# seanrjohnson/protein_gibbs_sampler

Measured on AMD Instinct MI355X. Metric: sampled positions/sec (whole node), ESM-1b L=256 B=256 Gibbs, higher is better.
Workload: dtype bf16

## Files before the change

protein_gibbs_sampler_amd/csrc/attention.hip:

```cpp
#include <stdlib.h>

#include "kernels.h"

PG_OPS_BEGIN

typedef __attribute__((ext_vector_type(8))) __bf16 bf16x8;
typedef __attribute__((ext_vector_type(4))) float f32x4;
typedef __attribute__((ext_vector_type(2))) float f32x2;

typedef short v4s __attribute__((ext_vector_type(4)));

#ifdef PG_ATT_PROF
__device__ unsigned long long* pg_att_prof;
#define PG_T(slot, i)                                                                                              \
  do {                                                                                                             \
    if ((slot) < 8 && (threadIdx.x & 63) == 0)                                                                     \
      pg_att_prof[(((size_t)blockIdx.x * 4 + (threadIdx.x >> 6)) * 8 + (slot)) * 8 + (i)] = __builtin_readcyclecounter(); \
  } while (0)
#else
#define PG_T(slot, i)
#endif

template <int MAXKB, bool PADMASK, bool BIASKV = false, bool SPLIT = false>
__global__ __launch_bounds__(256, (MAXKB <= 18 ? 2 : 1)) void attention_kernel(const bf16_t* __restrict__ qkv, bf16_t* __restrict__ ctx, int T,
                                                       int H, int ld_qkv_, int ld_ctx_, int k_off, int v_off,
                                                       SeqLayout sl, const int32_t* __restrict__ key_tok, int pad_idx,
                                                       const bf16_t* __restrict__ bias_kv, int split_from = 0, int split = 1) {
  __shared__ __attribute__((aligned(16))) char smem[2 * MAXKB * 16 * 128 + (PADMASK ? MAXKB * 16 : 0)];
  char* Ks = smem;
  char* Vs = smem + MAXKB * 16 * 128;
  char* padf = smem + 2 * MAXKB * 16 * 128;

  const int tid = threadIdx.x, lane = tid & 63, wave = tid >> 6;
  PG_T(7, 0);
  int pair = blockIdx.x, qb_first = wave, qb_step = 4;
  if (SPLIT && (int)blockIdx.x >= split_from) {
    const int u = blockIdx.x - split_from;
    pair = split_from + u / split;
    qb_first = u % split + split * wave;
    qb_step = 4 * split;
  }
  const int seq = pair / H, h = pair % H;
  const size_t row0 = (size_t)(seq / sl.inner_count) * sl.outer_rows + (size_t)(seq % sl.inner_count) * sl.inner_rows;
  const size_t ld_qkv = (size_t)ld_qkv_ * sl.row_step, ld_ctx = (size_t)ld_ctx_ * sl.row_step;
  const bf16_t* base = qkv + row0 * ld_qkv_ + h * 64;
  const int Tk = T + (BIASKV ? 1 : 0);
  constexpr int nkc = MAXKB / 2;
  constexpr int tpad = MAXKB * 16;

  {
    constexpr int NIT = (MAXKB * 16 * 8 + 255) / 256;
    uint4 kreg[NIT], vreg[NIT];
#pragma unroll
    for (int it = 0; it < NIT; ++it) {
      const int i = tid + it * 256;
      const int row = i >> 3, c = i & 7;
      kreg[it] = make_uint4(0, 0, 0, 0);
      vreg[it] = make_uint4(0, 0, 0, 0);
      if (i < tpad * 8 && row < T) {
        kreg[it] = *(const uint4*)(base + (size_t)row * ld_qkv + k_off + c * 8);
        vreg[it] = *(const uint4*)(base + (size_t)row * ld_qkv + v_off + c * 8);
      } else if (BIASKV && row == T) {
        kreg[it] = *(const uint4*)(bias_kv + h * 64 + c * 8);
        vreg[it] = *(const uint4*)(bias_kv + (H + h) * 64 + c * 8);
      }
    }
#pragma unroll
    for (int it = 0; it < NIT; ++it) {
      const int i = tid + it * 256;
      if (i < tpad * 8) {
        const int row = i >> 3, c = i & 7;
        *(uint4*)(Ks + row * 128 + ((c ^ (row & 7)) << 4)) = kreg[it];
        *(uint4*)(Vs + row * 128 + ((c ^ (row & 7)) << 4)) = vreg[it];
      }
    }
  }
  if (PADMASK) {
    for (int key = tid; key < MAXKB * 16; key += 256)
      padf[key] = (key < T && key_tok[row0 + (size_t)key * sl.row_step] == pad_idx) ? 1 : 0;
  }
  PG_T(7, 1);
  __syncthreads();
  PG_T(7, 2);

  const int fr = lane & 15, fq = lane >> 4;
  const int nqb = (T + 15) >> 4;
  bf16x8 qf[2], qn[2];
  auto load_q = [&](int qb, bf16x8 (&dst)[2]) {
    int qrow = qb * 16 + fr;
    if (qrow >= T) qrow = T - 1;
#pragma unroll
    for (int kk = 0; kk < 2; ++kk) dst[kk] = *(const bf16x8*)(base + (size_t)qrow * ld_qkv + kk * 32 + fq * 8);
  };
  if (qb_first < nqb) load_q(qb_first, qf);
  for (int qb = qb_first; qb < nqb; qb += qb_step) {
    if (qb + qb_step < nqb) load_q(qb + qb_step, qn);
    PG_T(qb >> 2, 0);

    f32x4 st[MAXKB];
    {
      constexpr int CH = (MAXKB % 6 == 0) ? 6 : (MAXKB % 4 == 0 ? 4 : 2);
      bf16x8 kbuf[2][CH][2];
      auto load_chunk = [&](int ch, bf16x8 (&dst)[CH][2]) {
#pragma unroll
        for (int u = 0; u < CH; ++u) {
#if defined(PG_ATT_PROF) && PG_ATT_ABL == 1
          const int krow = (ch * CH + (u > 0 ? 0 : u)) * 16 + fr;
          if (u > 0) { dst[u][0] = dst[0][0]; dst[u][1] = dst[0][1]; continue; }
#else
          const int krow = (ch * CH + u) * 16 + fr;
#endif
#pragma unroll
          for (int kk = 0; kk < 2; ++kk) dst[u][kk] = *(const bf16x8*)(Ks + krow * 128 + (((kk * 4 + fq) ^ (krow & 7)) << 4));
        }
      };
      load_chunk(0, kbuf[0]);
#pragma unroll
      for (int ch = 0; ch < MAXKB / CH; ++ch) {
        if (ch + 1 < MAXKB / CH) load_chunk(ch + 1, kbuf[(ch + 1) & 1]);
        __builtin_amdgcn_sched_barrier(0);
#pragma unroll
        for (int u = 0; u < CH; ++u)
          st[ch * CH + u] = mfma_op16(kbuf[ch & 1][u][0], qf[0], (f32x4){0.f, 0.f, 0.f, 0.f});
#pragma unroll
        for (int u = 0; u < CH; ++u)
          st[ch * CH + u] = mfma_op16(kbuf[ch & 1][u][1], qf[1], st[ch * CH + u]);
        __builtin_amdgcn_sched_barrier(0);
      }
    }
    PG_T(qb >> 2, 1);
    float mx = -3.0e38f;
    int tl = Tk - fq * 4;
    asm volatile("" : "+v"(tl));
#pragma unroll
    for (int kb = MAXKB > 6 ? MAXKB - 6 : 0; kb < MAXKB; ++kb)
      if ((kb + 1) * 16 > Tk) {
#pragma unroll
        for (int r = 0; r < 4; ++r)
          if (kb * 16 + r >= tl) st[kb][r] = -3.0e38f;
      }
#pragma unroll
    for (int kb = 0; kb < MAXKB; ++kb)
#pragma unroll
      for (int r = 0; r < 4; ++r) mx = fmaxf(mx, st[kb][r]);
    if (PADMASK) {
      const float fill = sl.row_step == 1 ? -3.0e38f : -10000.0f;
      mx = -3.0e38f;
#pragma unroll
      for (int kb = 0; kb < MAXKB; ++kb) {
        const uint32_t f4 = *(const uint32_t*)(padf + kb * 16 + fq * 4);
#pragma unroll
        for (int r = 0; r < 4; ++r) {
          if ((f4 >> (8 * r)) & 0xffu) st[kb][r] = fill;
          mx = fmaxf(mx, st[kb][r]);
        }
      }
    }
    mx = rows4_max(mx);
    const f32x2 l2e = {1.44269504088896341f, 1.44269504088896341f};
    const float mneg1 = -mx * 1.44269504088896341f;
    const f32x2 mneg = {mneg1, mneg1};
    f32x2 sum2 = {0.f, 0.f};
#pragma unroll
    for (int kb = 0; kb < MAXKB; ++kb) {
      const f32x2 a = __builtin_elementwise_fma((f32x2){st[kb][0], st[kb][1]}, l2e, mneg);
      const f32x2 b = __builtin_elementwise_fma((f32x2){st[kb][2], st[kb][3]}, l2e, mneg);
      const f32x2 ea = {__builtin_amdgcn_exp2f(a[0]), __builtin_amdgcn_exp2f(a[1])};
      const f32x2 eb = {__builtin_amdgcn_exp2f(b[0]), __builtin_amdgcn_exp2f(b[1])};
      st[kb] = (f32x4){ea[0], ea[1], eb[0], eb[1]};
      sum2 += ea;
      sum2 += eb;
    }
    float sum = sum2[0] + sum2[1];
    sum = rows4_sum(sum);
    const float inv = 1.0f / sum;
    PG_T(qb >> 2, 2);

    f32x4 o[4];
#pragma unroll
    for (int db = 0; db < 4; ++db) o[db] = (f32x4){0.f, 0.f, 0.f, 0.f};
    {
      union VF { bf16x8 v; uint2 h[2]; };
      VF vbuf[3][4];
      auto load_v = [&](int c, VF (&dst)[4]) {
#pragma unroll
        for (int db = 0; db < 4; ++db) {
#if defined(PG_ATT_PROF) && PG_ATT_ABL == 2
          if (db > 0) { dst[db] = dst[0]; continue; }
#endif
#pragma unroll
          for (int hh = 0; hh < 2; ++hh) {
            const int krow = (2 * c + hh) * 16 + fq * 4 + (fr >> 2);
            const int dcol = db * 16 + (fr & 3) * 4;
            const char* a = Vs + krow * 128 + (((dcol >> 3) ^ (krow & 7)) << 4) + ((dcol >> 2) & 1) * 8;
            const v4s t = __builtin_amdgcn_ds_read_tr16_b64_v4i16((v4s __attribute__((address_space(3)))*)(
                (__attribute__((address_space(3))) char*)a));
            dst[db].h[hh] = __builtin_bit_cast(uint2, t);
          }
        }
      };
      load_v(0, vbuf[0]);
      if (nkc > 1) load_v(1, vbuf[1]);
#pragma unroll
      for (int c = 0; c < nkc; ++c) {
        if (c + 2 < nkc) load_v(c + 2, vbuf[(c + 2) % 3]);
        union { bf16x8 v; uint32_t u[4]; } pf;
        const f32x4 lo = st[2 * c], hi = st[2 * c + 1];
        pf.u[0] = pack_op2(lo[0], lo[1]);
        pf.u[1] = pack_op2(lo[2], lo[3]);
        pf.u[2] = pack_op2(hi[0], hi[1]);
        pf.u[3] = pack_op2(hi[2], hi[3]);
        __builtin_amdgcn_sched_barrier(0);
#pragma unroll
        for (int db = 0; db < 4; ++db) o[db] = mfma_op16(vbuf[c % 3][db].v, pf.v, o[db]);
        __builtin_amdgcn_sched_barrier(0);
      }
    }
    PG_T(qb >> 2, 3);
    const int q = qb * 16 + fr;
    if (q < T) {
      bf16_t* dst = ctx + row0 * ld_ctx_ + (size_t)q * ld_ctx + h * 64 + fq * 4;
#pragma unroll
      for (int db = 0; db < 4; ++db) {
        uint2 p;
        p.x = pack_op2(o[db][0] * inv, o[db][1] * inv);
        p.y = pack_op2(o[db][2] * inv, o[db][3] * inv);
        *(uint2*)(dst + db * 16) = p;
      }
    }
    qf[0] = qn[0];
    qf[1] = qn[1];
    PG_T(qb >> 2, 4);
  }
  PG_T(7, 3);
}

template <int MAXKB, int OCC, bool PADMASK, bool BIASKV>
__global__ __launch_bounds__(256, OCC) void attention_long_kernel(const bf16_t* __restrict__ qkv, bf16_t* __restrict__ ctx, int T,
                                                               int H, int ld_qkv_, int ld_ctx_, int k_off, int v_off,
                                                               SeqLayout sl, int n_qchunk, const int32_t* __restrict__ key_tok_,
                                                               int pad_idx, const bf16_t* __restrict__ bias_kv_) {
  const int32_t* __restrict__ key_tok = PADMASK ? key_tok_ : nullptr;
  const bf16_t* __restrict__ bias_kv = BIASKV ? bias_kv_ : nullptr;
  constexpr int tpad = MAXKB * 16, nkc = MAXKB / 2;
  __shared__ __attribute__((aligned(16))) char smem[2 * tpad * 128 + (PADMASK ? tpad : 0)];
  char* Ks = smem;
  char* Vs = smem + tpad * 128;
  char* padf = smem + 2 * tpad * 128;
  const int tid = threadIdx.x, lane = tid & 63, wave = tid >> 6;
  const int qc = blockIdx.x % n_qchunk, sh = blockIdx.x / n_qchunk;
  const int seq = sh / H, h = sh % H;
  const size_t row0 = (size_t)(seq / sl.inner_count) * sl.outer_rows + (size_t)(seq % sl.inner_count) * sl.inner_rows;
  const size_t ld_qkv = (size_t)ld_qkv_ * sl.row_step, ld_ctx = (size_t)ld_ctx_ * sl.row_step;
  const bf16_t* base = qkv + row0 * ld_qkv_ + h * 64;
  const int fr = lane & 15, fq = lane >> 4;
  const int q0 = qc * 64 + wave * 16;
  const bool active = q0 < T;
  bf16x8 qf[2];
  {
    int qrow = q0 + fr;
    if (qrow >= T) qrow = T - 1;
#pragma unroll
    for (int kk = 0; kk < 2; ++kk) qf[kk] = *(const bf16x8*)(base + (size_t)qrow * ld_qkv + kk * 32 + fq * 8);
  }
  f32x4 o[4];
#pragma unroll
  for (int db = 0; db < 4; ++db) o[db] = (f32x4){0.f, 0.f, 0.f, 0.f};
  float m = -3.0e38f, l = 0.f;
  constexpr float LOG2E = 1.44269504088896341f;
  const int Tk = T + (bias_kv ? 1 : 0);

  for (int k0 = 0; k0 < Tk; k0 += tpad) {
    __syncthreads();
    {
      constexpr int NIT = (tpad * 8 + 255) / 256;
      uint4 kreg[NIT], vreg[NIT];
#pragma unroll
      for (int it = 0; it < NIT; ++it) {
        const int i = tid + it * 256, row = i >> 3, c = i & 7;
        kreg[it] = make_uint4(0, 0, 0, 0);
        vreg[it] = make_uint4(0, 0, 0, 0);
        if (i < tpad * 8 && k0 + row < T) {
          kreg[it] = *(const uint4*)(base + (size_t)(k0 + row) * ld_qkv + k_off + c * 8);
          vreg[it] = *(const uint4*)(base + (size_t)(k0 + row) * ld_qkv + v_off + c * 8);
        } else if (bias_kv && k0 + row == T) {
          kreg[it] = *(const uint4*)(bias_kv + h * 64 + c * 8);
          vreg[it] = *(const uint4*)(bias_kv + (H + h) * 64 + c * 8);
        }
      }
#pragma unroll
      for (int it = 0; it < NIT; ++it) {
        const int i = tid + it * 256, row = i >> 3, c = i & 7;
        if (i < tpad * 8) {
          *(uint4*)(Ks + row * 128 + ((c ^ (row & 7)) << 4)) = kreg[it];
          *(uint4*)(Vs + row * 128 + ((c ^ (row & 7)) << 4)) = vreg[it];
        }
      }
    }
    if (PADMASK) {
      for (int key = tid; key < tpad; key += 256)
        padf[key] = (k0 + key < T && key_tok[row0 + (size_t)(k0 + key) * sl.row_step] == pad_idx) ? 1 : 0;
    }
    __syncthreads();
    if (!active) continue;
    f32x4 st[MAXKB];
#pragma unroll
    for (int kb = 0; kb < MAXKB; ++kb) {
      st[kb] = (f32x4){0.f, 0.f, 0.f, 0.f};
      const int krow = kb * 16 + fr;
#pragma unroll
      for (int kk = 0; kk < 2; ++kk) {
        const bf16x8 kf = *(const bf16x8*)(Ks + krow * 128 + (((kk * 4 + fq) ^ (krow & 7)) << 4));
        st[kb] = mfma_op16(kf, qf[kk], st[kb]);
      }
    }
    float tmax = -3.0e38f;
    const int tl = Tk - k0 - fq * 4;
#pragma unroll
    for (int kb = 0; kb < MAXKB; ++kb)
#pragma unroll
      for (int r = 0; r < 4; ++r) {
        if (kb * 16 + r >= tl) st[kb][r] = -3.0e38f;
        tmax = fmaxf(tmax, st[kb][r]);
      }
    if (PADMASK) {
      const float fill = sl.row_step == 1 ? -3.0e38f : -10000.0f;
      tmax = -3.0e38f;
#pragma unroll
      for (int kb = 0; kb < MAXKB; ++kb) {
        const uint32_t f4 = *(const uint32_t*)(padf + kb * 16 + fq * 4);
#pragma unroll
        for (int r = 0; r < 4; ++r) {
          if ((f4 >> (8 * r)) & 0xffu) st[kb][r] = fill;
          tmax = fmaxf(tmax, st[kb][r]);
        }
      }
    }
    tmax = rows4_max(tmax);
    const float mn = fmaxf(m, tmax);
    const float alpha = __builtin_amdgcn_exp2f((m - mn) * LOG2E);
    const float mneg = -mn * LOG2E;
    float psum = 0.f;
#pragma unroll
    for (int kb = 0; kb < MAXKB; ++kb)
#pragma unroll
      for (int r = 0; r < 4; ++r) {
        const float e = __builtin_amdgcn_exp2f(fmaf(st[kb][r], LOG2E, mneg));
        st[kb][r] = e;
        psum += e;
      }
    psum = rows4_sum(psum);
    l = l * alpha + psum;
    m = mn;
#pragma unroll
    for (int db = 0; db < 4; ++db) {
      o[db][0] *= alpha; o[db][1] *= alpha; o[db][2] *= alpha; o[db][3] *= alpha;
    }
#pragma unroll
    for (int c = 0; c < nkc; ++c) {
      union { bf16x8 v; uint32_t u[4]; } pf;
      const f32x4 lo = st[2 * c], hi = st[2 * c + 1];
      pf.u[0] = pack_op2(lo[0], lo[1]);
      pf.u[1] = pack_op2(lo[2], lo[3]);
      pf.u[2] = pack_op2(hi[0], hi[1]);
      pf.u[3] = pack_op2(hi[2], hi[3]);
#pragma unroll
      for (int db = 0; db < 4; ++db) {
        union { bf16x8 v; uint2 h2[2]; } vf;
#pragma unroll
        for (int hh = 0; hh < 2; ++hh) {
          const int krow = (2 * c + hh) * 16 + fq * 4 + (fr >> 2);
          const int dcol = db * 16 + (fr & 3) * 4;
          const char* a = Vs + krow * 128 + (((dcol >> 3) ^ (krow & 7)) << 4) + ((dcol >> 2) & 1) * 8;
          vf.h2[hh] = __builtin_bit_cast(uint2, __builtin_amdgcn_ds_read_tr16_b64_v4i16((v4s __attribute__((address_space(3)))*)(
                                                    (__attribute__((address_space(3))) char*)a)));
        }
        o[db] = mfma_op16(vf.v, pf.v, o[db]);
      }
    }
  }
  const int q = q0 + fr;
  if (active && q < T) {
    const float inv = 1.0f / l;
    bf16_t* dst = ctx + row0 * ld_ctx_ + (size_t)q * ld_ctx + h * 64 + fq * 4;
#pragma unroll
    for (int db = 0; db < 4; ++db) {
      uint2 p;
      p.x = pack_op2(o[db][0] * inv, o[db][1] * inv);
      p.y = pack_op2(o[db][2] * inv, o[db][3] * inv);
      *(uint2*)(dst + db * 16) = p;
    }
  }
}

int launch_attention_bf16(hipStream_t s, const bf16_t* qkv, bf16_t* ctx, int B, int T, int H, int ld_qkv, int ld_ctx,
                          int k_off, int v_off, const int32_t* key_tok, int pad_idx, const bf16_t* bias_kv) {
  SeqLayout sl = {1, T, 0, 1};
  return launch_attention_seq_bf16(s, qkv, ctx, B, T, H, ld_qkv, ld_ctx, k_off, v_off, sl, key_tok, pad_idx, bias_kv);
}

int launch_attention_seq_bf16(hipStream_t s, const bf16_t* qkv, bf16_t* ctx, int64_t n_seq, int T, int H, int ld_qkv,
                              int ld_ctx, int k_off, int v_off, SeqLayout sl, const int32_t* key_tok, int pad_idx,
                              const bf16_t* bias_kv) {
  if (n_seq == 0) return 0;
  if (n_seq * H > 0x7fffffff) return fail(1, "attention: too many sequences");
  dim3 grid((unsigned)(n_seq * H)), block(256);
  static const int split_on = [] { const char* e = getenv("PGIBBS_ATTN_SPLIT"); return e ? atoi(e) : 1; }();
  static const int n_cu = [] { hipDeviceProp_t p; int d = 0; (void)hipGetDevice(&d); return hipGetDeviceProperties(&p, d) == hipSuccess ? p.multiProcessorCount : 256; }();
  int split_from = 0, split = 1;
  if (split_on && !key_tok && !bias_kv && sl.row_step == 1 && T >= 64 && T <= 576) {
    const int kb = (((T + 15) / 16) + 1) & ~1;
    const long pairs = n_seq * H, slots = (long)n_cu * (kb <= 20 ? 2 : 1);
    const long rem = pairs % slots;
    const int nqb = (T + 15) / 16;
    int sp = rem ? (int)(slots / rem) : 1;
    if (sp > 4) sp = 4;
    if (sp > nqb / 4) sp = nqb / 4;
    if (sp >= 2) {
      split = sp;
      split_from = (int)(pairs - rem);
      grid = dim3((unsigned)(split_from + rem * sp));
    }
  }
#define PG_ATT_SPLIT_LAUNCH(KB) hipLaunchKernelGGL((attention_kernel<KB, false, false, true>), grid, block, 0, s, qkv, ctx, T, H, ld_qkv, ld_ctx, k_off, v_off, sl, key_tok, pad_idx, bias_kv, split_from, split)
#define PG_ATT(KB)                                                                                             \
  else if (Tk <= KB * 16) {                                                                                    \
    if (bias_kv && key_tok) hipLaunchKernelGGL((attention_kernel<KB, true, true>), grid, block, 0, s, qkv, ctx, T, H, ld_qkv, ld_ctx, k_off, v_off, sl, key_tok, pad_idx, bias_kv); \
    else if (bias_kv) hipLaunchKernelGGL((attention_kernel<KB, false, true>), grid, block, 0, s, qkv, ctx, T, H, ld_qkv, ld_ctx, k_off, v_off, sl, key_tok, pad_idx, bias_kv); \
    else if (key_tok) hipLaunchKernelGGL((attention_kernel<KB, true>), grid, block, 0, s, qkv, ctx, T, H, ld_qkv, ld_ctx, k_off, v_off, sl, key_tok, pad_idx, bias_kv); \
    else if (split > 1) PG_ATT_SPLIT_LAUNCH(KB);                                                               \
    else hipLaunchKernelGGL((attention_kernel<KB, false>), grid, block, 0, s, qkv, ctx, T, H, ld_qkv, ld_ctx, k_off, v_off, sl, key_tok, pad_idx, bias_kv); \
  }
  const int Tk = T + (bias_kv ? 1 : 0);
  static const int fine_ladder = [] { const char* e = getenv("PGIBBS_ATTN_LADDER"); return e ? atoi(e) : 1; }();
  if (T <= 0) return fail(1, "attention: empty sequence");
#define PG_ATT_PLAIN(KB)                                                                                       \
  else if (fine_ladder && !bias_kv && Tk <= KB * 16) {                                                         \
    if (key_tok) hipLaunchKernelGGL((attention_kernel<KB, true>), grid, block, 0, s, qkv, ctx, T, H, ld_qkv, ld_ctx, k_off, v_off, sl, key_tok, pad_idx, bias_kv); \
    else if (split > 1) PG_ATT_SPLIT_LAUNCH(KB);                                                               \
    else hipLaunchKernelGGL((attention_kernel<KB, false>), grid, block, 0, s, qkv, ctx, T, H, ld_qkv, ld_ctx, k_off, v_off, sl, key_tok, pad_idx, bias_kv); \
  }
  PG_ATT(2) PG_ATT(4) PG_ATT_PLAIN(6) PG_ATT(8) PG_ATT_PLAIN(10) PG_ATT(12) PG_ATT_PLAIN(14) PG_ATT_PLAIN(16) PG_ATT(18)
  PG_ATT_PLAIN(20) PG_ATT_PLAIN(22) PG_ATT(24) PG_ATT_PLAIN(26) PG_ATT_PLAIN(28) PG_ATT(30) PG_ATT_PLAIN(32) PG_ATT_PLAIN(34) PG_ATT(36)
#undef PG_ATT_PLAIN
#undef PG_ATT
#undef PG_ATT_SPLIT_LAUNCH
  else {
    const int n_qchunk = (T + 63) / 64;
    if (n_seq * H * n_qchunk > 0x7fffffff) return fail(1, "attention: too many sequences");
    const dim3 g((unsigned)(n_seq * H * n_qchunk));
#define PG_ATT_LONG(P, B) hipLaunchKernelGGL((attention_long_kernel<18, 2, P, B>), g, block, 0, s, qkv, ctx, T, H, ld_qkv, ld_ctx, k_off, v_off, sl, n_qchunk, key_tok, pad_idx, bias_kv)
    if (key_tok && bias_kv) PG_ATT_LONG(true, true);
    else if (key_tok) PG_ATT_LONG(true, false);
    else if (bias_kv) PG_ATT_LONG(false, true);
    else PG_ATT_LONG(false, false);
#undef PG_ATT_LONG
  }
  PG_HIP(hipGetLastError());
  return 0;
}

PG_OPS_END
```

Baseline: 72010.

## Process two query blocks per wave in attention to reuse K/V fragment loads

Refactors the attention body into a templated pass that handles NQ query blocks at once, and adds a PAIR kernel variant in which each wave computes two 16-row query blocks per pass. Each K and V fragment read from LDS then feeds two MFMAs. The next pair's Q loads are issued after the score computation. The pair path is the default for unmasked, no-bias sequences with 14 to 28 key blocks, which includes L=256. In exchange it roughly doubles the score and accumulator registers, which risks spills or lower occupancy (launch bounds are adjusted for this), and it interacts with the existing split-block scheduling.

```diff
diff --git a/protein_gibbs_sampler_amd/csrc/attention.hip b/protein_gibbs_sampler_amd/csrc/attention.hip
--- a/protein_gibbs_sampler_amd/csrc/attention.hip
+++ b/protein_gibbs_sampler_amd/csrc/attention.hip
@@ -21,8 +21,183 @@
 #define PG_T(slot, i)
 #endif
 
-template <int MAXKB, bool PADMASK, bool BIASKV = false, bool SPLIT = false>
-__global__ __launch_bounds__(256, (MAXKB <= 18 ? 2 : 1)) void attention_kernel(const bf16_t* __restrict__ qkv, bf16_t* __restrict__ ctx, int T,
+template <int MAXKB, bool PADMASK, bool BIASKV, int NQ, class AfterS>
+__device__ __forceinline__ void attention_pass(const char* Ks, const char* Vs, const char* padf, bf16x8 (&qf)[2][2], const int (&qb)[2],
+                                               int slot, int T, int Tk, float padfill, bf16_t* ctx_head, size_t ld_ctx,
+                                               AfterS after_s) {
+  const int lane = threadIdx.x & 63, fr = lane & 15, fq = lane >> 4;
+  constexpr int nkc = MAXKB / 2;
+  PG_T(slot, 0);
+
+  f32x4 st[NQ][MAXKB];
+  {
+#if defined(PG_ATT_PROF) && defined(PG_ATT_PAIR_CH)
+    constexpr int CH = NQ == 2 ? (MAXKB == 18 ? PG_ATT_PAIR_CH : 2) : ((MAXKB % 6 == 0) ? 6 : (MAXKB % 4 == 0 ? 4 : 2));
+#else
+    constexpr int CH = NQ == 2 ? (MAXKB % 6 == 0 ? 3 : 2) : ((MAXKB % 6 == 0) ? 6 : (MAXKB % 4 == 0 ? 4 : 2));
+#endif
+    static_assert(MAXKB % CH == 0, "whole chunks");
+    bf16x8 kbuf[2][CH][2];
+    auto load_chunk = [&](int ch, bf16x8 (&dst)[CH][2]) {
+#pragma unroll
+      for (int u = 0; u < CH; ++u) {
+#if defined(PG_ATT_PROF) && PG_ATT_ABL == 1
+        const int krow = (ch * CH + (u > 0 ? 0 : u)) * 16 + fr;
+        if (u > 0) { dst[u][0] = dst[0][0]; dst[u][1] = dst[0][1]; continue; }
+#else
+        const int krow = (ch * CH + u) * 16 + fr;
+#endif
+#pragma unroll
+        for (int kk = 0; kk < 2; ++kk) dst[u][kk] = *(const bf16x8*)(Ks + krow * 128 + (((kk * 4 + fq) ^ (krow & 7)) << 4));
+      }
+    };
+    load_chunk(0, kbuf[0]);
+#pragma unroll
+    for (int ch = 0; ch < MAXKB / CH; ++ch) {
+      if (ch + 1 < MAXKB / CH) load_chunk(ch + 1, kbuf[(ch + 1) & 1]);
+      __builtin_amdgcn_sched_barrier(0);
+#pragma unroll
+      for (int u = 0; u < CH; ++u)
+#pragma unroll
+        for (int n = 0; n < NQ; ++n)
+          st[n][ch * CH + u] = mfma_op16(kbuf[ch & 1][u][0], qf[n][0], (f32x4){0.f, 0.f, 0.f, 0.f});
+#pragma unroll
+      for (int u = 0; u < CH; ++u)
+#pragma unroll
+        for (int n = 0; n < NQ; ++n)
+          st[n][ch * CH + u] = mfma_op16(kbuf[ch & 1][u][1], qf[n][1], st[n][ch * CH + u]);
+      __builtin_amdgcn_sched_barrier(0);
+    }
+  }
+  PG_T(slot, 1);
+  after_s();
+  float mx[NQ];
+  int tl = Tk - fq * 4;
+  asm volatile("" : "+v"(tl));
+#pragma unroll
+  for (int n = 0; n < NQ; ++n) {
+    mx[n] = -3.0e38f;
+#pragma unroll
+    for (int kb = MAXKB > 6 ? MAXKB - 6 : 0; kb < MAXKB; ++kb)
+      if ((kb + 1) * 16 > Tk) {
+#pragma unroll
+        for (int r = 0; r < 4; ++r)
+          if (kb * 16 + r >= tl) st[n][kb][r] = -3.0e38f;
+      }
+#pragma unroll
+    for (int kb = 0; kb < MAXKB; ++kb)
+#pragma unroll
+      for (int r = 0; r < 4; ++r) mx[n] = fmaxf(mx[n], st[n][kb][r]);
+    if (PADMASK) {
+      mx[n] = -3.0e38f;
+#pragma unroll
+      for (int kb = 0; kb < MAXKB; ++kb) {
+        const uint32_t f4 = *(const uint32_t*)(padf + kb * 16 + fq * 4);
+#pragma unroll
+        for (int r = 0; r < 4; ++r) {
+          if ((f4 >> (8 * r)) & 0xffu) st[n][kb][r] = padfill;
+          mx[n] = fmaxf(mx[n], st[n][kb][r]);
+        }
+      }
+    }
+    mx[n] = rows4_max(mx[n]);
+  }
+  const f32x2 l2e = {1.44269504088896341f, 1.44269504088896341f};
+  f32x2 mneg[NQ], sum2[NQ];
+#pragma unroll
+  for (int n = 0; n < NQ; ++n) {
+    const float mneg1 = -mx[n] * 1.44269504088896341f;
+    mneg[n] = (f32x2){mneg1, mneg1};
+    sum2[n] = (f32x2){0.f, 0.f};
+  }
+#pragma unroll
+  for (int kb = 0; kb < MAXKB; ++kb)
+#pragma unroll
+    for (int n = 0; n < NQ; ++n) {
+      const f32x2 a = __builtin_elementwise_fma((f32x2){st[n][kb][0], st[n][kb][1]}, l2e, mneg[n]);
+      const f32x2 b = __builtin_elementwise_fma((f32x2){st[n][kb][2], st[n][kb][3]}, l2e, mneg[n]);
+      const f32x2 ea = {__builtin_amdgcn_exp2f(a[0]), __builtin_amdgcn_exp2f(a[1])};
+      const f32x2 eb = {__builtin_amdgcn_exp2f(b[0]), __builtin_amdgcn_exp2f(b[1])};
+      st[n][kb] = (f32x4){ea[0], ea[1], eb[0], eb[1]};
+      sum2[n] += ea;
+      sum2[n] += eb;
+    }
+  float inv[NQ];
+#pragma unroll
+  for (int n = 0; n < NQ; ++n) {
+    float sum = sum2[n][0] + sum2[n][1];
+    sum = rows4_sum(sum);
+    inv[n] = 1.0f / sum;
+  }
+  PG_T(slot, 2);
+
+  f32x4 o[NQ][4];
+#pragma unroll
+  for (int n = 0; n < NQ; ++n)
+#pragma unroll
+    for (int db = 0; db < 4; ++db) o[n][db] = (f32x4){0.f, 0.f, 0.f, 0.f};
+  {
+    constexpr int VD = (NQ == 2 && MAXKB == 20) ? 2 : 3;
+    union VF { bf16x8 v; uint2 h[2]; };
+    VF vbuf[VD][4];
+    auto load_v = [&](int c, VF (&dst)[4]) {
+#pragma unroll
+      for (int db = 0; db < 4; ++db) {
+#if defined(PG_ATT_PROF) && PG_ATT_ABL == 2
+        if (db > 0) { dst[db] = dst[0]; continue; }
+#endif
+#pragma unroll
+        for (int hh = 0; hh < 2; ++hh) {
+          const int krow = (2 * c + hh) * 16 + fq * 4 + (fr >> 2);
+          const int dcol = db * 16 + (fr & 3) * 4;
+          const char* a = Vs + krow * 128 + (((dcol >> 3) ^ (krow & 7)) << 4) + ((dcol >> 2) & 1) * 8;
+          const v4s t = __builtin_amdgcn_ds_read_tr16_b64_v4i16((v4s __attribute__((address_space(3)))*)(
+              (__attribute__((address_space(3))) char*)a));
+          dst[db].h[hh] = __builtin_bit_cast(uint2, t);
+        }
+      }
+    };
+    load_v(0, vbuf[0]);
+    if (VD > 2 && nkc > 1) load_v(1, vbuf[1]);
+#pragma unroll
+    for (int c = 0; c < nkc; ++c) {
+      if (c + VD - 1 < nkc) load_v(c + VD - 1, vbuf[(c + VD - 1) % VD]);
+      union { bf16x8 v; uint32_t u[4]; } pf[NQ];
+#pragma unroll
+      for (int n = 0; n < NQ; ++n) {
+        const f32x4 lo = st[n][2 * c], hi = st[n][2 * c + 1];
+        pf[n].u[0] = pack_op2(lo[0], lo[1]);
+        pf[n].u[1] = pack_op2(lo[2], lo[3]);
+        pf[n].u[2] = pack_op2(hi[0], hi[1]);
+        pf[n].u[3] = pack_op2(hi[2], hi[3]);
+      }
+      __builtin_amdgcn_sched_barrier(0);
+#pragma unroll
+      for (int db = 0; db < 4; ++db)
+#pragma unroll
+        for (int n = 0; n < NQ; ++n) o[n][db] = mfma_op16(vbuf[c % VD][db].v, pf[n].v, o[n][db]);
+      __builtin_amdgcn_sched_barrier(0);
+    }
+  }
+  PG_T(slot, 3);
+#pragma unroll
+  for (int n = 0; n < NQ; ++n) {
+    const int q = qb[n] * 16 + fr;
+    if (q < T) {
+      bf16_t* dst = ctx_head + (size_t)q * ld_ctx + fq * 4;
+#pragma unroll
+      for (int db = 0; db < 4; ++db) {
+        uint2 p;
+        p.x = pack_op2(o[n][db][0] * inv[n], o[n][db][1] * inv[n]);
+        p.y = pack_op2(o[n][db][2] * inv[n], o[n][db][3] * inv[n]);
+        *(uint2*)(dst + db * 16) = p;
+      }
+    }
+  }
+}
+
+template <int MAXKB, bool PADMASK, bool BIASKV = false, bool SPLIT = false, bool PAIR = false>
+__global__ __launch_bounds__(256, (MAXKB <= (PAIR ? 20 : 18) ? 2 : 1)) void attention_kernel(const bf16_t* __restrict__ qkv, bf16_t* __restrict__ ctx, int T,
                                                        int H, int ld_qkv_, int ld_ctx_, int k_off, int v_off,
                                                        SeqLayout sl, const int32_t* __restrict__ key_tok, int pad_idx,
                                                        const bf16_t* __restrict__ bias_kv, int split_from = 0, int split = 1) {
@@ -45,8 +220,21 @@
   const size_t ld_qkv = (size_t)ld_qkv_ * sl.row_step, ld_ctx = (size_t)ld_ctx_ * sl.row_step;
   const bf16_t* base = qkv + row0 * ld_qkv_ + h * 64;
   const int Tk = T + (BIASKV ? 1 : 0);
-  constexpr int nkc = MAXKB / 2;
   constexpr int tpad = MAXKB * 16;
+
+  const int fr = lane & 15, fq = lane >> 4;
+  const int nqb = (T + 15) >> 4;
+  bf16x8 qf[2][2];
+  auto load_q = [&](int qb, bf16x8 (&dst)[2]) {
+    int qrow = qb * 16 + fr;
+    if (qrow >= T) qrow = T - 1;
+#pragma unroll
+    for (int kk = 0; kk < 2; ++kk) dst[kk] = *(const bf16x8*)(base + (size_t)qrow * ld_qkv + kk * 32 + fq * 8);
+  };
+  if (PAIR) {
+    if (qb_first < nqb) load_q(qb_first, qf[0]);
+    if (qb_first + qb_step < nqb) load_q(qb_first + qb_step, qf[1]);
+  }
 
   {
     constexpr int NIT = (MAXKB * 16 * 8 + 255) / 256;
@@ -83,154 +271,34 @@
   __syncthreads();
   PG_T(7, 2);
 
-  const int fr = lane & 15, fq = lane >> 4;
-  const int nqb = (T + 15) >> 4;
-  bf16x8 qf[2], qn[2];
-  auto load_q = [&](int qb, bf16x8 (&dst)[2]) {
-    int qrow = qb * 16 + fr;
-    if (qrow >= T) qrow = T - 1;
-#pragma unroll
-    for (int kk = 0; kk < 2; ++kk) dst[kk] = *(const bf16x8*)(base + (size_t)qrow * ld_qkv + kk * 32 + fq * 8);
-  };
-  if (qb_first < nqb) load_q(qb_first, qf);
-  for (int qb = qb_first; qb < nqb; qb += qb_step) {
-    if (qb + qb_step < nqb) load_q(qb + qb_step, qn);
-    PG_T(qb >> 2, 0);
-
-    f32x4 st[MAXKB];
-    {
-      constexpr int CH = (MAXKB % 6 == 0) ? 6 : (MAXKB % 4 == 0 ? 4 : 2);
-      bf16x8 kbuf[2][CH][2];
-      auto load_chunk = [&](int ch, bf16x8 (&dst)[CH][2]) {
-#pragma unroll
-        for (int u = 0; u < CH; ++u) {
-#if defined(PG_ATT_PROF) && PG_ATT_ABL == 1
-          const int krow = (ch * CH + (u > 0 ? 0 : u)) * 16 + fr;
-          if (u > 0) { dst[u][0] = dst[0][0]; dst[u][1] = dst[0][1]; continue; }
-#else
-          const int krow = (ch * CH + u) * 16 + fr;
-#endif
-#pragma unroll
-          for (int kk = 0; kk < 2; ++kk) dst[u][kk] = *(const bf16x8*)(Ks + krow * 128 + (((kk * 4 + fq) ^ (krow & 7)) << 4));
-        }
-      };
-      load_chunk(0, kbuf[0]);
-#pragma unroll
-      for (int ch = 0; ch < MAXKB / CH; ++ch) {
-        if (ch + 1 < MAXKB / CH) load_chunk(ch + 1, kbuf[(ch + 1) & 1]);
-        __builtin_amdgcn_sched_barrier(0);
-#pragma unroll
-        for (int u = 0; u < CH; ++u)
-          st[ch * CH + u] = mfma_op16(kbuf[ch & 1][u][0], qf[0], (f32x4){0.f, 0.f, 0.f, 0.f});
-#pragma unroll
-        for (int u = 0; u < CH; ++u)
-          st[ch * CH + u] = mfma_op16(kbuf[ch & 1][u][1], qf[1], st[ch * CH + u]);
-        __builtin_amdgcn_sched_barrier(0);
-      }
-    }
-    PG_T(qb >> 2, 1);
-    float mx = -3.0e38f;
-    int tl = Tk - fq * 4;
-    asm volatile("" : "+v"(tl));
-#pragma unroll
-    for (int kb = MAXKB > 6 ? MAXKB - 6 : 0; kb < MAXKB; ++kb)
-      if ((kb + 1) * 16 > Tk) {
-#pragma unroll
-        for (int r = 0; r < 4; ++r)
-          if (kb * 16 + r >= tl) st[kb][r] = -3.0e38f;
-      }
-#pragma unroll
-    for (int kb = 0; kb < MAXKB; ++kb)
-#pragma unroll
-      for (int r = 0; r < 4; ++r) mx = fmaxf(mx, st[kb][r]);
-    if (PADMASK) {
-      const float fill = sl.row_step == 1 ? -3.0e38f : -10000.0f;
-      mx = -3.0e38f;
-#pragma unroll
-      for (int kb = 0; kb < MAXKB; ++kb) {
-        const uint32_t f4 = *(const uint32_t*)(padf + kb * 16 + fq * 4);
-#pragma unroll
-        for (int r = 0; r < 4; ++r) {
-          if ((f4 >> (8 * r)) & 0xffu) st[kb][r] = fill;
-          mx = fmaxf(mx, st[kb][r]);
-        }
-      }
-    }
-    mx = rows4_max(mx);
-    const f32x2 l2e = {1.44269504088896341f, 1.44269504088896341f};
-    const float mneg1 = -mx * 1.44269504088896341f;
-    const f32x2 mneg = {mneg1, mneg1};
-    f32x2 sum2 = {0.f, 0.f};
-#pragma unroll
-    for (int kb = 0; kb < MAXKB; ++kb) {
-      const f32x2 a = __builtin_elementwise_fma((f32x2){st[kb][0], st[kb][1]}, l2e, mneg);
-      const f32x2 b = __builtin_elementwise_fma((f32x2){st[kb][2], st[kb][3]}, l2e, mneg);
-      const f32x2 ea = {__builtin_amdgcn_exp2f(a[0]), __builtin_amdgcn_exp2f(a[1])};
-      const f32x2 eb = {__builtin_amdgcn_exp2f(b[0]), __builtin_amdgcn_exp2f(b[1])};
-      st[kb] = (f32x4){ea[0], ea[1], eb[0], eb[1]};
-      sum2 += ea;
-      sum2 += eb;
-    }
-    float sum = sum2[0] + sum2[1];
-    sum = rows4_sum(sum);
-    const float inv = 1.0f / sum;
-    PG_T(qb >> 2, 2);
-
-    f32x4 o[4];
-#pragma unroll
-    for (int db = 0; db < 4; ++db) o[db] = (f32x4){0.f, 0.f, 0.f, 0.f};
-    {
-      union VF { bf16x8 v; uint2 h[2]; };
-      VF vbuf[3][4];
-      auto load_v = [&](int c, VF (&dst)[4]) {
-#pragma unroll
-        for (int db = 0; db < 4; ++db) {
-#if defined(PG_ATT_PROF) && PG_ATT_ABL == 2
-          if (db > 0) { dst[db] = dst[0]; continue; }
-#endif
-#pragma unroll
-          for (int hh = 0; hh < 2; ++hh) {
-            const int krow = (2 * c + hh) * 16 + fq * 4 + (fr >> 2);
-            const int dcol = db * 16 + (fr & 3) * 4;
-            const char* a = Vs + krow * 128 + (((dcol >> 3) ^ (krow & 7)) << 4) + ((dcol >> 2) & 1) * 8;
-            const v4s t = __builtin_amdgcn_ds_read_tr16_b64_v4i16((v4s __attribute__((address_space(3)))*)(
-                (__attribute__((address_space(3))) char*)a));
-            dst[db].h[hh] = __builtin_bit_cast(uint2, t);
-          }
-        }
-      };
-      load_v(0, vbuf[0]);
-      if (nkc > 1) load_v(1, vbuf[1]);
-#pragma unroll
-      for (int c = 0; c < nkc; ++c) {
-        if (c + 2 < nkc) load_v(c + 2, vbuf[(c + 2) % 3]);
-        union { bf16x8 v; uint32_t u[4]; } pf;
-        const f32x4 lo = st[2 * c], hi = st[2 * c + 1];
-        pf.u[0] = pack_op2(lo[0], lo[1]);
-        pf.u[1] = pack_op2(lo[2], lo[3]);
-        pf.u[2] = pack_op2(hi[0], hi[1]);
-        pf.u[3] = pack_op2(hi[2], hi[3]);
-        __builtin_amdgcn_sched_barrier(0);
-#pragma unroll
-        for (int db = 0; db < 4; ++db) o[db] = mfma_op16(vbuf[c % 3][db].v, pf.v, o[db]);
-        __builtin_amdgcn_sched_barrier(0);
-      }
-    }
-    PG_T(qb >> 2, 3);
-    const int q = qb * 16 + fr;
-    if (q < T) {
-      bf16_t* dst = ctx + row0 * ld_ctx_ + (size_t)q * ld_ctx + h * 64 + fq * 4;
-#pragma unroll
-      for (int db = 0; db < 4; ++db) {
-        uint2 p;
-        p.x = pack_op2(o[db][0] * inv, o[db][1] * inv);
-        p.y = pack_op2(o[db][2] * inv, o[db][3] * inv);
-        *(uint2*)(dst + db * 16) = p;
-      }
-    }
-    qf[0] = qn[0];
-    qf[1] = qn[1];
-    PG_T(qb >> 2, 4);
+  const float padfill = sl.row_step == 1 ? -3.0e38f : -10000.0f;
+  bf16_t* ctx_head = ctx + row0 * ld_ctx_ + h * 64;
+  if (!PAIR) {
+    if (qb_first < nqb) load_q(qb_first, qf[0]);
+    bf16x8 qn[2];
+    for (int qb = qb_first; qb < nqb; qb += qb_step) {
+      if (qb + qb_step < nqb) load_q(qb + qb_step, qn);
+      attention_pass<MAXKB, PADMASK, BIASKV, 1>(Ks, Vs, padf, qf, {qb, 0}, qb >> 2, T, Tk, padfill, ctx_head, ld_ctx, [] {});
+      qf[0][0] = qn[0];
+      qf[0][1] = qn[1];
+      PG_T(qb >> 2, 4);
+    }
+  } else {
+    int slot = 0;
+    for (int qb = qb_first; qb < nqb; ++slot) {
+      if (qb + qb_step < nqb) {
+        const int nx = qb + 2 * qb_step;
+        attention_pass<MAXKB, PADMASK, BIASKV, 2>(Ks, Vs, padf, qf, {qb, qb + qb_step}, slot, T, Tk, padfill, ctx_head, ld_ctx, [&] {
+          if (nx < nqb) load_q(nx, qf[0]);
+          if (nx + qb_step < nqb) load_q(nx + qb_step, qf[1]);
+        });
+        qb = nx;
+      } else {
+        attention_pass<MAXKB, PADMASK, BIASKV, 1>(Ks, Vs, padf, qf, {qb, 0}, slot, T, Tk, padfill, ctx_head, ld_ctx, [] {});
+        qb += qb_step;
+      }
+      PG_T(slot, 4);
+    }
   }
   PG_T(7, 3);
 }
@@ -393,6 +461,12 @@
   }
 }
 
+constexpr int kPairMaxKB = 28;
+template <int KB, class... Args>
+static void launch_attention_pair(dim3 grid, hipStream_t s, Args... args) {
+  if constexpr (KB <= kPairMaxKB) hipLaunchKernelGGL((attention_kernel<KB, false, false, true, true>), grid, dim3(256), 0, s, args...);
+}
+
 int launch_attention_bf16(hipStream_t s, const bf16_t* qkv, bf16_t* ctx, int B, int T, int H, int ld_qkv, int ld_ctx,
                           int k_off, int v_off, const int32_t* key_tok, int pad_idx, const bf16_t* bias_kv) {
   SeqLayout sl = {1, T, 0, 1};
@@ -422,12 +496,18 @@
       grid = dim3((unsigned)(split_from + rem * sp));
     }
   }
+  static const int pair_on = [] { const char* e = getenv("PGIBBS_ATTN_PAIR"); return e ? atoi(e) : 1; }();
+  const int pair_min_kb = pair_on >= 2 ? 2 : 14;
+  const bool pair = pair_on && !key_tok && !bias_kv && sl.row_step == 1;
+  if (pair && split == 1) split_from = (int)grid.x;
 #define PG_ATT_SPLIT_LAUNCH(KB) hipLaunchKernelGGL((attention_kernel<KB, false, false, true>), grid, block, 0, s, qkv, ctx, T, H, ld_qkv, ld_ctx, k_off, v_off, sl, key_tok, pad_idx, bias_kv, split_from, split)
+#define PG_ATT_PAIR_LAUNCH(KB) launch_attention_pair<KB>(grid, s, qkv, ctx, T, H, ld_qkv, ld_ctx, k_off, v_off, sl, key_tok, pad_idx, bias_kv, split_from, split)
 #define PG_ATT(KB)                                                                                             \
   else if (Tk <= KB * 16) {                                                                                    \
     if (bias_kv && key_tok) hipLaunchKernelGGL((attention_kernel<KB, true, true>), grid, block, 0, s, qkv, ctx, T, H, ld_qkv, ld_ctx, k_off, v_off, sl, key_tok, pad_idx, bias_kv); \
     else if (bias_kv) hipLaunchKernelGGL((attention_kernel<KB, false, true>), grid, block, 0, s, qkv, ctx, T, H, ld_qkv, ld_ctx, k_off, v_off, sl, key_tok, pad_idx, bias_kv); \
     else if (key_tok) hipLaunchKernelGGL((attention_kernel<KB, true>), grid, block, 0, s, qkv, ctx, T, H, ld_qkv, ld_ctx, k_off, v_off, sl, key_tok, pad_idx, bias_kv); \
+    else if (pair && KB >= pair_min_kb && KB <= kPairMaxKB) PG_ATT_PAIR_LAUNCH(KB);                          \
     else if (split > 1) PG_ATT_SPLIT_LAUNCH(KB);                                                               \
     else hipLaunchKernelGGL((attention_kernel<KB, false>), grid, block, 0, s, qkv, ctx, T, H, ld_qkv, ld_ctx, k_off, v_off, sl, key_tok, pad_idx, bias_kv); \
   }
@@ -437,6 +517,7 @@
 #define PG_ATT_PLAIN(KB)                                                                                       \
   else if (fine_ladder && !bias_kv && Tk <= KB * 16) {                                                         \
     if (key_tok) hipLaunchKernelGGL((attention_kernel<KB, true>), grid, block, 0, s, qkv, ctx, T, H, ld_qkv, ld_ctx, k_off, v_off, sl, key_tok, pad_idx, bias_kv); \
+    else if (pair && KB >= pair_min_kb && KB <= kPairMaxKB) PG_ATT_PAIR_LAUNCH(KB);                          \
     else if (split > 1) PG_ATT_SPLIT_LAUNCH(KB);                                                               \
     else hipLaunchKernelGGL((attention_kernel<KB, false>), grid, block, 0, s, qkv, ctx, T, H, ld_qkv, ld_ctx, k_off, v_off, sl, key_tok, pad_idx, bias_kv); \
   }
@@ -445,6 +526,7 @@
 #undef PG_ATT_PLAIN
 #undef PG_ATT
 #undef PG_ATT_SPLIT_LAUNCH
+#undef PG_ATT_PAIR_LAUNCH
   else {
     const int n_qchunk = (T + 63) / 64;
     if (n_seq * H * n_qchunk > 0x7fffffff) return fail(1, "attention: too many sequences");
```

Result: no change. 72360, median of 6 (+0.5%).
